# Freebirdgo/MapReduce_Rust

Hardware: AMD Instinct MI355X
Metric: word-count input GB/s (whole node) at 1/2/4/8 MI355X + % of HBM roofline (higher is better)
Workload: dtype u8

## Files before the change

mapreduce_rust_amd/csrc/k_keys.hip:

```cpp
#include <algorithm>
#include <type_traits>

#include "mrg_device.h"
#include "mrg_internal.h"

namespace {

inline dim3 grid_for(uint64_t n, int b = 256) { return dim3((unsigned)((n + b - 1) / b)); }

template <int WG>
__device__ __forceinline__ uint64_t wg_append(unsigned long long *counter, bool pred, uint32_t *s_w,
                                              unsigned long long *s_base) {
    const uint64_t m = __ballot(pred);
    const uint32_t wv = threadIdx.x >> 6, lane = __lane_id();
    if (lane == 0) s_w[wv] = (uint32_t)__popcll(m);
    __syncthreads();
    if (threadIdx.x == 0) {
        uint32_t run = 0;
        for (int w = 0; w < WG / 64; ++w) {
            const uint32_t c = s_w[w];
            s_w[w] = run;
            run += c;
        }
        *s_base = run ? atomicAdd(counter, (unsigned long long)run) : 0ull;
    }
    __syncthreads();
    return *s_base + s_w[wv] + (uint64_t)__popcll(m & mrg_lanemask_lt());
}

constexpr int BA_WG = 1024;
constexpr int BA_NW = BA_WG / 64;
template <bool IDX, bool C32>
constexpr uint32_t ba_cap() { return IDX ? 4096u : (C32 ? 6912u : 6112u); }
constexpr int BA_PROBE = 64;
constexpr int BA_U = 8;
template <bool C32>
constexpr int ba_maxreg() { return C32 ? 512 : 2048; }
constexpr uint32_t BA_QN = 64;
template <bool IDX, bool C32>
constexpr bool ba_queue() { return !IDX && C32; }

#define GASK __attribute__((address_space(1)))
template <class T>
__device__ __forceinline__ GASK T *gk(T *p) {
    return (GASK T *)p;
}
typedef uint64_t u64x2k __attribute__((ext_vector_type(2)));
typedef uint32_t u32x3k __attribute__((ext_vector_type(3), aligned(4)));

__device__ __forceinline__ uint32_t ba_hash(uint64_t a, uint64_t b, uint32_t d, uint32_t hash_bits) {
    uint32_t h = mrg_key_hash32(a, b, d);
    if (hash_bits && hash_bits < 32) h &= (1u << hash_bits) - 1u;
    return h;
}

struct alignas(16) BaKey {
    unsigned long long a, b;
};

template <bool IDX, bool C32>
__device__ __forceinline__ uint32_t ba_slot(uint32_t h) {
    return (((h >> (32 - MRG_NBUCKET_LOG2 - 16)) & 0xFFFFu) * ba_cap<IDX, C32>()) >> 16;
}

template <bool IDX, bool C32, class CT>
__device__ __forceinline__ bool ba_add_from(BaKey *key, CT *cnt, unsigned int *doc, uint64_t a,
                                            uint64_t b, uint32_t d, uint64_t c, uint32_t h, BaKey first) {
    constexpr uint32_t CAP = ba_cap<IDX, C32>();
    uint32_t slot = ba_slot<IDX, C32>(h);
    BaKey kn = first;
    for (int p = 0; p < BA_PROBE; ++p) {
        const BaKey k = kn;
        uint32_t nxt = slot + 1u + (uint32_t)p;
        if (nxt >= CAP) nxt -= CAP;
        kn = key[nxt];
        const bool dk = !IDX || doc[slot] == d;
        if (k.a == a && k.b == b && dk) {
            atomicAdd(&cnt[slot], (CT)c);
            return true;
        }
        if (k.a == MRG_EMPTY_K0 || (k.a == a && (k.b == MRG_EMPTY_K1 || (IDX && k.b == b)))) {
            const unsigned long long x = atomicCAS(&key[slot].a, MRG_EMPTY_K0, (unsigned long long)a);
            if (x == MRG_EMPTY_K0 || x == a) {
                const unsigned long long y = atomicCAS(&key[slot].b, MRG_EMPTY_K1, (unsigned long long)b);
                if (y == MRG_EMPTY_K1 || y == b) {
                    bool ok = true;
                    if (IDX) {
                        const unsigned int z = atomicCAS(&doc[slot], MRG_EMPTY_DOC, d);
                        ok = (z == MRG_EMPTY_DOC || z == d);
                    }
                    if (ok) {
                        atomicAdd(&cnt[slot], (CT)c);
                        return true;
                    }
                }
            }
        }
        slot = nxt;
    }
    return false;
}

template <bool IDX, bool C32, class CT>
__device__ __forceinline__ bool ba_add(BaKey *key, CT *cnt, unsigned int *doc, uint64_t a,
                                       uint64_t b, uint32_t d, uint64_t c, uint32_t h) {
    return ba_add_from<IDX, C32>(key, cnt, doc, a, b, d, c, h, key[ba_slot<IDX, C32>(h)]);
}

#ifndef MRG_AGG_XCD
#define MRG_AGG_XCD 1
#endif
static_assert(MRG_NBUCKET % 8 == 0, "buckets spread over the 8 XCDs");
template <bool IDX, bool C32>
__global__ __launch_bounds__(BA_WG, 1) void k_bucket_agg(BucketArgs A) {
    constexpr uint32_t BA_CAP = ba_cap<IDX, C32>();
    using CT = typename std::conditional<C32, unsigned int, unsigned long long>::type;
    __shared__ BaKey s_key[BA_CAP];
    __shared__ CT s_cnt[BA_CAP];
    __shared__ unsigned int s_doc[IDX ? BA_CAP : 1];
    __shared__ uint32_t s_rn[ba_maxreg<C32>()];
    __shared__ uint32_t s_cs[ba_maxreg<C32>() + 1];
    __shared__ BaKey s_mq[ba_queue<IDX, C32>() ? BA_NW : 1][ba_queue<IDX, C32>() ? BA_QN : 1];
    const int tid = threadIdx.x, lane = tid & 63;
    const int wv = __builtin_amdgcn_readfirstlane(tid >> 6);
    for (int i = tid; i < (int)BA_CAP; i += BA_WG) {
        s_key[i] = BaKey{MRG_EMPTY_K0, MRG_EMPTY_K1};
        s_cnt[i] = 0;
        if (IDX) s_doc[i] = MRG_EMPTY_DOC;
    }
    const uint32_t nsub = A.nsub;
#if MRG_AGG_XCD
    const uint32_t g = blockIdx.x, slot = g / 8u;
    const uint32_t b = nsub > 1u ? (slot / nsub) * 8u + g % 8u : g % MRG_NBUCKET;
    const uint32_t jsub = nsub > 1u ? slot % nsub : g / MRG_NBUCKET;
#else
    const uint32_t b = blockIdx.x % MRG_NBUCKET, jsub = blockIdx.x / MRG_NBUCKET;
#endif
    auto mine = [&](uint32_t h) { return nsub <= 1u || (((h & 0xFFu) * nsub) >> 8) == jsub; };
    constexpr uint32_t RW = IDX ? 3u : 2u;
    const uint32_t cap = gk(A.bcap)[b];
    const uint32_t nreg = A.nreg;
    for (uint32_t r = tid; r < nreg; r += BA_WG) s_rn[r] = min(gk(A.bcount)[(uint64_t)r * MRG_NBUCKET + b], cap);
    __syncthreads();
    constexpr uint32_t CH = 64u * BA_U;
    if (wv == 0) {
        uint32_t run = 0;
        for (uint32_t r0 = 0; r0 < nreg; r0 += 64) {
            const uint32_t r = r0 + (uint32_t)lane;
            const uint32_t c = r < nreg ? (s_rn[r] + CH - 1u) / CH : 0u;
            uint32_t incl = c;
            for (int o = 1; o < 64; o <<= 1) {
                const uint32_t v = __shfl_up(incl, o);
                if (lane >= o) incl += v;
            }
            if (r < nreg) s_cs[r] = run + incl - c;
            run += (uint32_t)__builtin_amdgcn_readlane((int)incl, 63);
        }
        if (lane == 0) s_cs[nreg] = run;
    }
    __syncthreads();
    const uint32_t NC = s_cs[nreg];

    auto overflow = [&](bool ovf, uint64_t a, uint64_t c, uint32_t d, uint64_t n2) {
        const uint64_t j = mrg_wave_append(&A.counters[CNT_OVF2], ovf);
        if (ovf && j < A.ocap) {
            gk(A.ok0)[j] = a; gk(A.ok1)[j] = c; gk(A.ocnt)[j] = (uint32_t)n2;
            if (IDX) gk(A.odoc)[j] = d;
        }
    };

    const GASK uint8_t *pool = reinterpret_cast<const GASK uint8_t *>(gk(A.pool)) + A.rbase[b] * MRG_TAIL_BYTES(IDX);
    struct Chunk {
        u64x2k k[BA_U];
        uint32_t d[IDX ? BA_U : 1];
    };
    auto chunk_pos = [&](uint32_t k, uint32_t &r) -> uint32_t {
        while (s_cs[r + 1] <= k) ++r;
        return (k - s_cs[r]) * CH;
    };
    auto load_chunk = [&](uint32_t r, uint32_t off, Chunk &X) {
        const uint32_t n = s_rn[r];
        const GASK uint8_t *src = pool + (uint64_t)r * cap * MRG_TAIL_BYTES(IDX);
#pragma unroll
        for (int k = 0; k < BA_U; ++k) {
            const uint32_t i = min(off + 64u * k + (uint32_t)lane, n - 1u);
            if (IDX) {
                const GASK uint64_t *rec = reinterpret_cast<const GASK uint64_t *>(src) + (uint64_t)i * 3;
                X.k[k] = u64x2k{rec[0], rec[1]};
                X.d[k] = (uint32_t)rec[2];
            } else {
                const u32x3k v = __builtin_nontemporal_load(reinterpret_cast<const GASK u32x3k *>(src + (uint64_t)i * 12u));
                X.k[k] = u64x2k{(uint64_t)v.x | ((uint64_t)v.y << 32), (uint64_t)v.z << 32};
            }
        }
    };
    auto settle = [](Chunk &X) {
#pragma unroll
        for (int k = 0; k < BA_U; ++k) asm volatile("" : "+v"(X.k[k]));
        if (IDX)
            for (int k = 0; k < BA_U; ++k) asm volatile("" : "+v"(X.d[k]));
    };
    uint64_t abl_acc = 0;
    uint32_t qn = 0;
    auto drain = [&]() {
        if (!ba_queue<IDX, C32>() || qn == 0) return;
        const bool act = (uint32_t)lane < qn;
        const BaKey r = s_mq[ba_queue<IDX, C32>() ? wv : 0][act ? lane : 0];
        bool ovf = false;
        if (act) {
            const uint32_t h = ba_hash(r.a, r.b, MRG_EMPTY_DOC, A.hash_bits);
            ovf = !ba_add<IDX, C32>(s_key, s_cnt, s_doc, r.a, r.b, MRG_EMPTY_DOC, 1ull, h);
        }
        if (__any(ovf)) overflow(ovf, r.a, r.b, MRG_EMPTY_DOC, 1);
        qn = 0;
    };
    auto sum_chunk = [&](uint32_t r, uint32_t off, const Chunk &X) {
        const uint32_t n = s_rn[r];
        if (A.ablate) {
#pragma unroll
            for (int k = 0; k < BA_U; ++k) {
                const bool ok = off + 64u * k + (uint32_t)lane < n;
                const uint64_t a = X.k[k].x, c = X.k[k].y;
                const uint32_t d = IDX ? X.d[k] : MRG_EMPTY_DOC;
                abl_acc += ok ? ((A.ablate & 2u) ? (a ^ c) : (uint64_t)ba_hash(a, c, d, A.hash_bits)) : 0u;
            }
            return;
        }
        uint32_t hk[BA_U];
#pragma unroll
        for (int k = 0; k < BA_U; ++k) hk[k] = ba_hash(X.k[k].x, X.k[k].y, IDX ? X.d[k] : MRG_EMPTY_DOC, A.hash_bits);
        BaKey pre = s_key[ba_slot<IDX, C32>(hk[0])];
        if constexpr (ba_queue<IDX, C32>()) {
#pragma unroll
            for (int k = 0; k < BA_U; ++k) {
                const bool ok = off + 64u * k + (uint32_t)lane < n;
                const uint64_t a = X.k[k].x, c = X.k[k].y;
                const BaKey first = pre;
                if (k + 1 < BA_U) pre = s_key[ba_slot<IDX, C32>(hk[k + 1 < BA_U ? k + 1 : k])];
                const uint32_t h = hk[k];
                const bool me = ok && mine(h);
                const bool hit = me && first.a == a && first.b == c;
                if (hit) atomicAdd(&s_cnt[ba_slot<IDX, C32>(h)], (CT)1);
                const bool miss = me && !hit;
                const uint64_t mm = __ballot(miss);
                if (mm) {
                    const uint32_t m = (uint32_t)__builtin_popcountll(mm);
                    if (qn + m > BA_QN) drain();
                    if (miss) s_mq[wv][qn + (uint32_t)__builtin_popcountll(mm & mrg_lanemask_lt())] = BaKey{a, c};
                    qn += m;
                }
            }
            return;
        }
#pragma unroll
        for (int k = 0; k < BA_U; ++k) {
            const bool ok = off + 64u * k + (uint32_t)lane < n;
            const uint64_t a = X.k[k].x, c = X.k[k].y;
            const uint32_t d = IDX ? X.d[k] : MRG_EMPTY_DOC;
            const BaKey first = pre;
            if (k + 1 < BA_U) pre = s_key[ba_slot<IDX, C32>(hk[k + 1 < BA_U ? k + 1 : k])];
            bool ovf = false;
            const uint32_t h = hk[k];
            if (ok && mine(h)) ovf = !ba_add_from<IDX, C32>(s_key, s_cnt, s_doc, a, c, d, 1ull, h, first);
            if (__any(ovf)) overflow(ovf, a, c, d, 1);
        }
    };
    if (!(A.ablate & 4u)) {
        Chunk XA, XB;
        uint32_t kA = (uint32_t)wv, rA = 0, oA = 0;
        if (kA < NC) {
            oA = chunk_pos(kA, rA);
            load_chunk(rA, oA, XA);
        }
        while (kA < NC) {
            const uint32_t kB = kA + BA_NW;
            uint32_t rB = rA, oB = oA;
            if (kB < NC) oB = chunk_pos(kB, rB);
            settle(XA);
            load_chunk(rB, oB, XB);
            sum_chunk(rA, oA, XA);
            if (kB >= NC) break;
            kA = kB + BA_NW;
            rA = rB;
            if (kA < NC) oA = chunk_pos(kA, rA);
            else oA = oB;
            settle(XB);
            load_chunk(rA, oA, XA);
            sum_chunk(rB, oB, XB);
        }
    }
    drain();

    if (A.ablate && abl_acc == 0x9E3779B97F4A7C15ull) atomicAdd(&A.counters[CNT_OVF2], 1ull);
    {
        const uint32_t nrw = nreg > (uint32_t)wv ? (nreg - (uint32_t)wv + BA_NW - 1) / BA_NW : 0u;
        for (uint32_t l0 = 0; l0 < nrw; l0 += 64) {
            const uint32_t l = l0 + (uint32_t)lane;
            uint32_t lo = 0, cnt = 0;
            if (l < nrw) {
                const GASK uint32_t *fo = gk(A.foff) + (uint64_t)(wv + BA_NW * l) * (MRG_NBUCKET + 1);
                lo = fo[b];
                cnt = fo[b + 1] - lo;
            }
            uint32_t incl = cnt;
            for (int o = 1; o < 64; o <<= 1) {
                const uint32_t v = __shfl_up(incl, o);
                if (lane >= o) incl += v;
            }
            const uint32_t excl = incl - cnt;
            const uint32_t total = (uint32_t)__builtin_amdgcn_readlane((int)incl, 63);
            for (uint32_t e0 = 0; e0 < total; e0 += 256) {
                uint64_t a[4], c[4];
                uint32_t n2[4], d[4];
                bool ok[4];
#pragma unroll
                for (int u = 0; u < 4; ++u) {
                    const uint32_t e = e0 + 64u * u + (uint32_t)lane;
                    ok[u] = e < total;
                    uint32_t k = 0;
#pragma unroll
                    for (int st = 32; st > 0; st >>= 1)
                        if (__shfl(excl, (int)(k + st)) <= e) k += st;
                    const uint32_t rl = l0 + k;
                    const uint64_t at = (uint64_t)(wv + BA_NW * rl) * A.regcap + __shfl(lo, (int)k) + (e - __shfl(excl, (int)k));
                    a[u] = 0; c[u] = 0; n2[u] = 0; d[u] = MRG_EMPTY_DOC;
                    if (ok[u]) {
                        a[u] = gk(A.fk0)[at];
                        c[u] = gk(A.fk1)[at];
                        n2[u] = gk(A.fcnt)[at];
                        if (IDX) d[u] = gk(A.fdoc)[at];
                    }
                }
#pragma unroll
                for (int u = 0; u < 4; ++u) {
                    bool ovf = false;
                    if (ok[u]) {
                        const uint32_t h = ba_hash(a[u], c[u], d[u], A.hash_bits);
                        if (mine(h)) ovf = !ba_add<IDX, C32>(s_key, s_cnt, s_doc, a[u], c[u], d[u], n2[u], h);
                    }
                    if (__any(ovf)) overflow(ovf, a[u], c[u], d[u], n2[u]);
                }
            }
        }
    }
    if (!IDX) {
        const uint32_t cap16 = gk(A.bcap16)[b];
        const GASK uint64_t *p16 = gk(A.pool16) + 2ull * A.rbase16[b];
        for (uint32_t r = (uint32_t)wv; r < nreg; r += BA_NW) {
            const uint32_t n = min(gk(A.bcount16)[(uint64_t)r * MRG_NBUCKET + b], cap16);
            const GASK uint64_t *src = p16 + 2ull * r * cap16;
            for (uint32_t base = 0; base < n; base += 64) {
                const uint32_t i = base + (uint32_t)lane;
                bool ovf = false;
                uint64_t a = 0, c = 0;
                if (i < n) {
                    const u64x2k v = *reinterpret_cast<const GASK u64x2k *>(src + 2ull * i);
                    a = v.x;
                    c = v.y;
                    const uint32_t h = ba_hash(a, c, MRG_EMPTY_DOC, A.hash_bits);
                    if (mine(h)) ovf = !ba_add<IDX, C32>(s_key, s_cnt, s_doc, a, c, MRG_EMPTY_DOC, 1ull, h);
                }
                if (__any(ovf)) overflow(ovf, a, c, MRG_EMPTY_DOC, 1);
            }
        }
    }
    {
        const uint32_t n = min(gk(A.monext)[b], A.mocap);
        const GASK uint64_t *src = gk(A.movf) + (uint64_t)b * A.mocap * RW;
        for (uint32_t base = wv * 64u; base < n; base += BA_WG) {
            const uint32_t i = base + lane;
            bool ovf = false;
            uint64_t a = 0, c = 0;
            uint32_t d = MRG_EMPTY_DOC;
            if (i < n) {
                a = src[(uint64_t)i * RW];
                c = src[(uint64_t)i * RW + 1];
                if (IDX) d = (uint32_t)src[(uint64_t)i * RW + 2];
                const uint32_t h = ba_hash(a, c, d, A.hash_bits);
                if (mine(h)) ovf = !ba_add<IDX, C32>(s_key, s_cnt, s_doc, a, c, d, 1ull, h);
            }
            if (__any(ovf)) overflow(ovf, a, c, d, 1);
        }
    }
    __syncthreads();
    constexpr int NP = (int)((BA_CAP + BA_WG - 1) / BA_WG);
    constexpr int NPW = NP * BA_NW;
    static_assert(NPW <= 128, "one wave scans two entries per lane");
    __shared__ uint32_t s_po[NPW];
    __shared__ unsigned long long s_base;
#pragma unroll
    for (int pp = 0; pp < NP; ++pp) {
        const int i = pp * BA_WG + tid;
        const uint64_t m = __ballot(i < (int)BA_CAP && s_key[min(i, (int)BA_CAP - 1)].a != MRG_EMPTY_K0);
        if (lane == 0) s_po[pp * BA_NW + wv] = (uint32_t)__popcll(m);
    }
    __syncthreads();
    if (wv == 0) {
        const int e0 = 2 * lane, e1 = e0 + 1;
        const uint32_t c0 = e0 < NPW ? s_po[e0] : 0u, c1 = e1 < NPW ? s_po[e1] : 0u;
        uint32_t incl = c0 + c1;
        for (int o = 1; o < 64; o <<= 1) {
            const uint32_t v = __shfl_up(incl, o);
            if (lane >= o) incl += v;
        }
        const uint32_t ex = incl - c0 - c1;
        if (e0 < NPW) s_po[e0] = ex;
        if (e1 < NPW) s_po[e1] = ex + c0;
        const uint32_t tot = (uint32_t)__shfl((int)incl, 63);
        if (lane == 0) s_base = tot ? atomicAdd(&A.counters[CNT_KEYS], (unsigned long long)tot) : 0ull;
    }
    __syncthreads();
    const uint64_t kbase = s_base;
    for (int pp = 0; pp < NP; ++pp) {
        const int i = min(pp * BA_WG + tid, (int)BA_CAP - 1);
        const BaKey k = s_key[i];
        const bool full = pp * BA_WG + tid < (int)BA_CAP && k.a != MRG_EMPTY_K0;
        const uint64_t m = __ballot(full);
        const uint64_t j = kbase + s_po[pp * BA_NW + wv] + (uint64_t)__popcll(m & mrg_lanemask_lt());
        if (full && j < A.kcap) {
            gk(A.out.k0)[j] = k.a;
            gk(A.out.k1)[j] = k.b;
            gk(A.out.cnt)[j] = s_cnt[i];
            gk(A.out.doc)[j] = IDX ? s_doc[i] : MRG_EMPTY_DOC;
            const uint32_t L = mrg_short_len(k.a, k.b);
            gk(A.out.len)[j] = L;
            gk(A.out.hoff)[j] = MRG_NO_HEAP;
            if (A.n_reduce) gk(A.out.part)[j] = (uint32_t)(mrg_siphash_short(k.a, k.b, L) % (uint64_t)A.n_reduce);
        }
    }
}

__global__ __launch_bounds__(1024) void k_stage_scatter(const uint8_t *stage, uint32_t table_off, uint32_t nops) {
    const StageOp *ops = reinterpret_cast<const StageOp *>(stage + table_off);
    for (uint32_t k = 0; k < nops; ++k) {
        const StageOp op = ops[k];
        uint8_t *dst = reinterpret_cast<uint8_t *>(op.dst);
        const bool fill = op.src == 0xFFFFFFFFu;
        if (((op.dst | op.n) & 3u) == 0u) {
            const uint32_t f4 = op.fill * 0x01010101u;
            const uint32_t *src = reinterpret_cast<const uint32_t *>(stage + (fill ? 0u : op.src));
            for (uint32_t i = threadIdx.x; i < op.n / 4u; i += blockDim.x)
                reinterpret_cast<uint32_t *>(dst)[i] = fill ? f4 : src[i];
        } else {
            for (uint32_t i = threadIdx.x; i < op.n; i += blockDim.x) dst[i] = fill ? (uint8_t)op.fill : stage[op.src + i];
        }
        __syncthreads();
    }
}

__global__ void k_table_clear(TableArgs T, bool idx) {
    const uint64_t i = (uint64_t)blockIdx.x * blockDim.x + threadIdx.x;
    if (i >= T.cap) return;
    T.tk0[i] = MRG_EMPTY_K0;
    T.tk1[i] = MRG_EMPTY_K1;
    T.tcnt[i] = 0;
    if (idx) T.tdoc[i] = MRG_EMPTY_DOC;
}

__device__ __forceinline__ void table_add(const TableArgs &T, uint64_t a, uint64_t b, uint32_t d, uint64_t c,
                                          bool idx) {
    uint64_t h = mrg_key_mix(a, b, d);
    if (T.hash_bits) h &= (1ull << T.hash_bits) - 1u;
    uint64_t slot = (h ^ (h >> 31)) & (T.cap - 1);
    for (uint64_t probe = 0; probe < T.cap; ++probe) {
        const unsigned long long x =
            atomicCAS((unsigned long long *)&T.tk0[slot], MRG_EMPTY_K0, (unsigned long long)a);
        if (x == MRG_EMPTY_K0 || x == a) {
            const unsigned long long y =
                atomicCAS((unsigned long long *)&T.tk1[slot], MRG_EMPTY_K1, (unsigned long long)b);
            if (y == MRG_EMPTY_K1 || y == b) {
                bool ok = true;
                if (idx) {
                    const unsigned int z = atomicCAS(&T.tdoc[slot], MRG_EMPTY_DOC, d);
                    ok = (z == MRG_EMPTY_DOC || z == d);
                }
                if (ok) {
                    atomicAdd((unsigned long long *)&T.tcnt[slot], (unsigned long long)c);
                    return;
                }
            }
        }
        slot = (slot + probe + 1u) & (T.cap - 1);
    }
}

__global__ void k_table_insert(TableArgs T, const uint64_t *k0, const uint64_t *k1, const uint32_t *cnt,
                               const uint32_t *doc, uint64_t n, bool idx) {
    const uint64_t i = (uint64_t)blockIdx.x * blockDim.x + threadIdx.x;
    if (i >= n) return;
    table_add(T, k0[i], k1[i], idx ? doc[i] : MRG_EMPTY_DOC, cnt[i], idx);
}

__global__ void k_table_insert_x(TableArgs T, const XRec *x, uint64_t n, bool idx) {
    const uint64_t i = (uint64_t)blockIdx.x * blockDim.x + threadIdx.x;
    if (i >= n) return;
    const XRec r = x[i];
    if (r.len > 16u) return;
    table_add(T, r.a, r.b, idx ? r.v : MRG_EMPTY_DOC, idx ? 1ull : (uint64_t)r.v, idx);
}

__global__ void k_table_insert_l(TableArgs T, const LRec *x, uint64_t n, bool idx) {
    const uint64_t i = (uint64_t)blockIdx.x * blockDim.x + threadIdx.x;
    if (i >= n) return;
    const LRec r = x[i];
    if (r.len > 16u) return;
    table_add(T, r.k0, r.k1, idx ? r.doc : MRG_EMPTY_DOC, r.cnt, idx);
}

constexpr int TC_WG = 1024;
__global__ __launch_bounds__(TC_WG) void k_table_compact(TableArgs T, bool idx, KeySet out, unsigned long long *counter) {
    __shared__ uint32_t s_w[TC_WG / 64];
    __shared__ unsigned long long s_base;
    const uint64_t i = (uint64_t)blockIdx.x * blockDim.x + threadIdx.x;
    const bool full = i < T.cap && T.tk0[i] != MRG_EMPTY_K0;
    const uint64_t j = wg_append<TC_WG>(counter, full, s_w, &s_base);
    if (!full) return;
    const uint64_t a = T.tk0[i], b = T.tk1[i];
    out.k0[j] = a;
    out.k1[j] = b;
    out.cnt[j] = T.tcnt[i];
    out.doc[j] = idx ? T.tdoc[i] : MRG_EMPTY_DOC;
    out.len[j] = mrg_short_len(a, b);
    out.hoff[j] = MRG_NO_HEAP;
}

__global__ void k_partition(KeySet ks, const uint8_t *heap, uint64_t n, uint32_t n_reduce) {
    const uint64_t i = (uint64_t)blockIdx.x * blockDim.x + threadIdx.x;
    if (i >= n) return;
    const uint32_t L = ks.len[i];
    const uint64_t h = L <= 16u ? mrg_siphash_short(ks.k0[i], ks.k1[i], L) : mrg_siphash_bytes(heap + ks.hoff[i], L);
    ks.part[i] = (uint32_t)(h % (uint64_t)n_reduce);
}

__global__ void k_wide_counts(BucketArgs A, uint64_t *cnt) {
    const uint64_t s = (uint64_t)blockIdx.x * blockDim.x + threadIdx.x;
    const uint64_t nt = (uint64_t)A.nreg * MRG_NBUCKET;
    if (s < nt) {
        const uint32_t b = (uint32_t)(s / A.nreg), w = (uint32_t)(s % A.nreg);
        cnt[s] = min(A.bcount[(uint64_t)w * MRG_NBUCKET + b], A.bcap[b]);
    } else if (s < nt + A.nreg) {
        const uint64_t w = s - nt;
        cnt[s] = A.foff[w * (MRG_NBUCKET + 1) + MRG_NBUCKET];
    } else if (s < nt + A.nreg + MRG_NBUCKET) {
        const uint32_t b = (uint32_t)(s - nt - A.nreg);
        cnt[s] = min(A.monext[b], A.mocap);
    } else if (s < 2 * nt + A.nreg + MRG_NBUCKET) {
        const uint64_t s2 = s - nt - A.nreg - MRG_NBUCKET;
        const uint32_t b = (uint32_t)(s2 / A.nreg), w = (uint32_t)(s2 % A.nreg);
        cnt[s] = min(A.bcount16[(uint64_t)w * MRG_NBUCKET + b], A.bcap16[b]);
    }
}

__global__ void k_wide_gather(BucketArgs A, const uint64_t *off, uint32_t n_reduce, SortRec *out) {
    const uint64_t s = blockIdx.x;
    const uint64_t nt = (uint64_t)A.nreg * MRG_NBUCKET;
    const uint64_t o = off[s], n = off[s + 1] - o;
    for (uint64_t i = threadIdx.x; i < n; i += blockDim.x) {
        uint64_t k0, k1;
        uint32_t c = 1;
        if (s < nt) {
            const uint32_t b = (uint32_t)(s / A.nreg), w = (uint32_t)(s % A.nreg);
            const uint64_t j = A.rbase[b] + (uint64_t)w * A.bcap[b] + i;
            const uint32_t *rec = reinterpret_cast<const uint32_t *>(reinterpret_cast<const uint8_t *>(A.pool) + 12u * j);
            k0 = (uint64_t)rec[0] | ((uint64_t)rec[1] << 32);
            k1 = (uint64_t)rec[2] << 32;
        } else if (s >= nt + A.nreg + MRG_NBUCKET) {
            const uint64_t s2 = s - nt - A.nreg - MRG_NBUCKET;
            const uint32_t b = (uint32_t)(s2 / A.nreg), w = (uint32_t)(s2 % A.nreg);
            const uint64_t j = A.rbase16[b] + (uint64_t)w * A.bcap16[b] + i;
            k0 = A.pool16[2 * j];
            k1 = A.pool16[2 * j + 1];
        } else if (s < nt + A.nreg) {
            const uint64_t j = (s - nt) * A.regcap + i;
            k0 = A.fk0[j];
            k1 = A.fk1[j];
            c = A.fcnt[j];
        } else {
            const uint64_t b = s - nt - A.nreg;
            const uint64_t j = b * A.mocap + i;
            k0 = A.movf[2 * j];
            k1 = A.movf[2 * j + 1];
        }
        SortRec r;
        r.k0 = k0;
        r.k1 = k1;
        r.part = (uint32_t)(mrg_siphash_short(k0, k1, mrg_short_len(k0, k1)) % (uint64_t)n_reduce);
        r.doc = 0;
        r.idx = c;
        r.pad = 0;
        out[o + i] = r;
    }
}

__global__ void k_wide_heads(const SortRec *r, uint64_t n, uint64_t *head, uint64_t *cv) {
    const uint64_t i = (uint64_t)blockIdx.x * blockDim.x + threadIdx.x;
    if (i >= n) return;
    head[i] = (i == 0 || r[i].k0 != r[i - 1].k0 || r[i].k1 != r[i - 1].k1) ? 1u : 0u;
    cv[i] = r[i].idx;
}

__global__ void k_wide_keys(const SortRec *r, uint64_t n, const uint64_t *head, const uint64_t *E, KeySet ks,
                            uint64_t *F) {
    const uint64_t i = (uint64_t)blockIdx.x * blockDim.x + threadIdx.x;
    if (i >= n || !head[i]) return;
    const uint64_t k = E[i];
    ks.k0[k] = r[i].k0;
    ks.k1[k] = r[i].k1;
    ks.doc[k] = MRG_EMPTY_DOC;
    ks.len[k] = mrg_short_len(r[i].k0, r[i].k1);
    ks.part[k] = r[i].part;
    ks.hoff[k] = MRG_NO_HEAP;
    F[k] = i;
}

__global__ void k_wide_cnt(const uint64_t *F, uint64_t runs, uint64_t n, const uint64_t *C, uint64_t ctot, KeySet ks) {
    const uint64_t k = (uint64_t)blockIdx.x * blockDim.x + threadIdx.x;
    if (k >= runs) return;
    const uint64_t e = k + 1 < runs ? C[F[k + 1]] : ctot;
    ks.cnt[k] = e - C[F[k]];
}

__global__ void k_long_group(const uint64_t *fp, const uint32_t *idx, const uint32_t *doc, const uint8_t *heap,
                             const uint64_t *hoff, const uint32_t *flen, uint64_t n, uint32_t *rep) {
    const uint64_t i = (uint64_t)blockIdx.x * blockDim.x + threadIdx.x;
    if (i >= n) return;
    const uint32_t me = idx[i];
    const uint64_t f = fp[i];
    uint64_t g = 0, hi = i;
    while (g < hi) {
        const uint64_t mid = (g + hi) >> 1;
        if (fp[mid] < f) g = mid + 1; else hi = mid;
    }
    uint32_t r = me;
    const uint8_t *mk = heap + hoff[me];
    const uint32_t ml = flen[me];
    for (uint64_t j = g; j < i; ++j) {
        const uint32_t o = idx[j];
        if (flen[o] != ml || (doc && doc[o] != doc[me])) continue;
        const uint8_t *ok = heap + hoff[o];
        bool eq = true;
        for (uint32_t b = 0; b < ml && eq; ++b) eq = mk[b] == ok[b];
        if (eq) { r = o; break; }
    }
    rep[me] = r;
}

__global__ void k_long_count(const uint32_t *rep, const uint64_t *cnt_in, uint64_t n, unsigned long long *acc) {
    const uint64_t i = (uint64_t)blockIdx.x * blockDim.x + threadIdx.x;
    if (i >= n) return;
    atomicAdd(&acc[rep[i]], (unsigned long long)(cnt_in ? cnt_in[i] : 1u));
}

__global__ void k_long_emit(const uint32_t *rep, const uint64_t *k0, const uint64_t *k1, const uint32_t *flen,
                            const uint64_t *hoff, const uint32_t *doc, uint64_t n, const unsigned long long *acc,
                            KeySet out, unsigned long long *counter, bool idx) {
    const uint64_t i = (uint64_t)blockIdx.x * blockDim.x + threadIdx.x;
    const bool mine = i < n && rep[i] == (uint32_t)i;
    const uint64_t j = mrg_wave_append(counter, mine);
    if (!mine) return;
    out.k0[j] = k0[i];
    out.k1[j] = k1[i];
    out.cnt[j] = acc[i];
    out.doc[j] = idx ? doc[i] : MRG_EMPTY_DOC;
    out.len[j] = flen[i];
    out.hoff[j] = hoff[i];
}

__device__ __forceinline__ uint32_t seg_of(const uint64_t *seg_rec_end, uint32_t n_segs, uint64_t i) {
    uint32_t lo = 0, hi = n_segs - 1u;
    while (lo < hi) {
        const uint32_t mid = (lo + hi) >> 1;
        if (i < seg_rec_end[mid]) hi = mid;
        else lo = mid + 1u;
    }
    return lo;
}

__global__ void k_x_split_long(const XRec *x, uint64_t n, const uint64_t *seg_rec_end, const uint64_t *seg_heap_base,
                               uint32_t n_segs, LongItems li, unsigned long long *counter, bool idx) {
    const uint64_t i = (uint64_t)blockIdx.x * blockDim.x + threadIdx.x;
    const bool lng = i < n && x[i].len > 16u;
    const uint64_t j = mrg_wave_append(counter, lng);
    if (!lng) return;
    const XRec r = x[i];
    li.start[j] = seg_heap_base[seg_of(seg_rec_end, n_segs, i)] + r.a;
    li.rawlen[j] = r.len;
    li.doc[j] = idx ? r.v : MRG_EMPTY_DOC;
    li.cnt[j] = idx ? 1ull : r.b;
}

__global__ void k_l_split_long(const LRec *x, uint64_t n, const uint64_t *seg_rec_end, const uint64_t *seg_heap_base,
                               uint32_t n_segs, LongItems li, unsigned long long *counter) {
    const uint64_t i = (uint64_t)blockIdx.x * blockDim.x + threadIdx.x;
    const bool lng = i < n && x[i].len > 16u;
    const uint64_t j = mrg_wave_append(counter, lng);
    if (!lng) return;
    const LRec r = x[i];
    li.start[j] = seg_heap_base[seg_of(seg_rec_end, n_segs, i)] + r.heap;
    li.rawlen[j] = r.len;
    li.doc[j] = r.doc;
    li.cnt[j] = r.cnt;
}

constexpr int EXP_WG = 1024;
constexpr uint32_t EXP_MAXO = 256;

__global__ __launch_bounds__(EXP_WG) void k_export_count(KeySet ks, uint64_t n, uint32_t n_owners,
                                                         unsigned long long *rec_cnt, unsigned long long *heap_cnt,
                                                         bool idx, uint64_t vmax) {
    __shared__ unsigned long long s_rc[EXP_MAXO];
    __shared__ unsigned long long s_hc[EXP_MAXO];
    const bool lds = n_owners <= EXP_MAXO;
    if (lds)
        for (uint32_t o = threadIdx.x; o < n_owners; o += EXP_WG) {
            s_rc[o] = 0;
            s_hc[o] = 0;
        }
    __syncthreads();
    const uint64_t i = (uint64_t)blockIdx.x * blockDim.x + threadIdx.x;
    if (i < n) {
        const uint32_t o = ks.part[i] % n_owners;
        const uint32_t len = ks.len[i];
        const unsigned long long nr = mrg_xrec_per_key(ks.cnt[i], len, idx, vmax);
        if (lds) {
            atomicAdd(&s_rc[o], nr);
            if (len > 16u) atomicAdd(&s_hc[o], (unsigned long long)len);
        } else {
            atomicAdd(&rec_cnt[o], nr);
            if (len > 16u) atomicAdd(&heap_cnt[o], (unsigned long long)len);
        }
    }
    if (!lds) return;
    __syncthreads();
    for (uint32_t o = threadIdx.x; o < n_owners; o += EXP_WG) {
        if (s_rc[o]) atomicAdd(&rec_cnt[o], (unsigned long long)s_rc[o]);
        if (s_hc[o]) atomicAdd(&heap_cnt[o], s_hc[o]);
    }
}

__global__ __launch_bounds__(EXP_WG) void k_export_pack(KeySet ks, const uint8_t *heap, uint64_t n, uint32_t n_owners,
                                                        const uint64_t *rec_base, const uint64_t *heap_base,
                                                        unsigned long long *rec_cur, unsigned long long *heap_cur,
                                                        XRec *out, uint8_t *out_heap, bool idx, uint64_t vmax) {
    __shared__ unsigned long long s_rc[EXP_MAXO];
    __shared__ unsigned long long s_hc[EXP_MAXO], s_rb[EXP_MAXO], s_hb[EXP_MAXO];
    const bool lds = n_owners <= EXP_MAXO;
    if (lds)
        for (uint32_t o = threadIdx.x; o < n_owners; o += EXP_WG) {
            s_rc[o] = 0;
            s_hc[o] = 0;
        }
    __syncthreads();
    const uint64_t i = (uint64_t)blockIdx.x * blockDim.x + threadIdx.x;
    const bool act = i < n;
    uint32_t o = 0, len = 0;
    uint64_t cnt = 0, nr = 0;
    unsigned long long lr = 0, lh = 0;
    if (act) {
        o = ks.part[i] % n_owners;
        len = ks.len[i];
        cnt = ks.cnt[i];
        nr = mrg_xrec_per_key(cnt, len, idx, vmax);
        if (lds) {
            lr = atomicAdd(&s_rc[o], (unsigned long long)nr);
            if (len > 16u) lh = atomicAdd(&s_hc[o], (unsigned long long)len);
        } else {
            lr = atomicAdd(&rec_cur[o], (unsigned long long)nr);
            if (len > 16u) lh = atomicAdd(&heap_cur[o], (unsigned long long)len);
        }
    }
    if (lds) {
        __syncthreads();
        for (uint32_t q = threadIdx.x; q < n_owners; q += EXP_WG) {
            s_rb[q] = s_rc[q] ? atomicAdd(&rec_cur[q], (unsigned long long)s_rc[q]) : 0ull;
            s_hb[q] = s_hc[q] ? atomicAdd(&heap_cur[q], s_hc[q]) : 0ull;
        }
        __syncthreads();
        if (act) {
            lr += s_rb[o];
            lh += s_hb[o];
        }
    }
    if (!act) return;
    const uint64_t slot = rec_base[o] + lr;
    XRec r;
    r.len = len;
    if (len > 16u) {
        const uint8_t *src = heap + ks.hoff[i];
        uint8_t *dst = out_heap + heap_base[o] + lh;
        for (uint32_t b = 0; b < len; ++b) dst[b] = src[b];
        r.a = lh;
        r.b = idx ? 1ull : cnt;
        r.v = idx ? ks.doc[i] : MRG_EMPTY_DOC;
        out[slot] = r;
        return;
    }
    r.a = ks.k0[i];
    r.b = ks.k1[i];
    if (idx) {
        r.v = ks.doc[i];
        out[slot] = r;
        return;
    }
    for (uint64_t k = 0; k < nr; ++k) {
        const uint64_t c = cnt > vmax ? vmax : cnt;
        cnt -= c;
        r.v = (uint32_t)c;
        out[slot + k] = r;
    }
}

__global__ void k_make_sortrec(KeySet ks, uint64_t n, const uint32_t *doc_rank, SortRec *out, int carry) {
    const uint64_t i = (uint64_t)blockIdx.x * blockDim.x + threadIdx.x;
    if (i >= n) return;
    SortRec r;
    r.k0 = ks.k0[i];
    r.k1 = ks.k1[i];
    r.part = ks.part[i];
    r.doc = doc_rank ? doc_rank[ks.doc[i]] : 0u;
    r.idx = (uint32_t)i;
    r.pad = 0;
    if (carry) {
        const uint64_t c = ks.cnt[i];
        const uint32_t len = ks.len[i];
        r.doc = (uint32_t)c;
        r.pad = (len <= 16u ? len : 0xFFu) | ((uint32_t)(c >> 32) << 8);
    }
    out[i] = r;
}

template <class T>
__global__ void k_fill(T *p, T v, uint64_t n) {
    const uint64_t i = (uint64_t)blockIdx.x * blockDim.x + threadIdx.x;
    if (i < n) p[i] = v;
}
__global__ void k_iota(uint32_t *p, uint64_t n) {
    const uint64_t i = (uint64_t)blockIdx.x * blockDim.x + threadIdx.x;
    if (i < n) p[i] = (uint32_t)i;
}

}

void mrg_launch_stage_scatter(const uint8_t *d_stage, uint32_t table_off, uint32_t nops, hipStream_t s) {
    if (nops) hipLaunchKernelGGL(k_stage_scatter, dim3(1), dim3(1024), 0, s, d_stage, table_off, nops);
}

void mrg_launch_bucket_agg(const BucketArgs &a, bool indexer, bool count32, hipStream_t s) {
    const dim3 g(MRG_NBUCKET * std::max<uint32_t>(a.nsub, 1u));
    if (indexer) hipLaunchKernelGGL((k_bucket_agg<true, false>), g, dim3(BA_WG), 0, s, a);
    else if (count32) hipLaunchKernelGGL((k_bucket_agg<false, true>), g, dim3(BA_WG), 0, s, a);
    else hipLaunchKernelGGL((k_bucket_agg<false, false>), g, dim3(BA_WG), 0, s, a);
}

void mrg_launch_table_clear(const TableArgs &t, bool indexer, hipStream_t s) {
    hipLaunchKernelGGL(k_table_clear, grid_for(t.cap), dim3(256), 0, s, t, indexer);
}
void mrg_launch_table_insert(const TableArgs &t, const uint64_t *k0, const uint64_t *k1, const uint32_t *cnt32,
                             const uint32_t *doc, uint64_t n, bool indexer, hipStream_t s) {
    if (!n) return;
    hipLaunchKernelGGL(k_table_insert, grid_for(n), dim3(256), 0, s, t, k0, k1, cnt32, doc, n, indexer);
}
void mrg_launch_table_insert_x(const TableArgs &t, const XRec *x, uint64_t n, bool indexer, hipStream_t s) {
    if (!n) return;
    hipLaunchKernelGGL(k_table_insert_x, grid_for(n), dim3(256), 0, s, t, x, n, indexer);
}
void mrg_launch_table_insert_l(const TableArgs &t, const LRec *x, uint64_t n, bool indexer, hipStream_t s) {
    if (!n) return;
    hipLaunchKernelGGL(k_table_insert_l, grid_for(n), dim3(256), 0, s, t, x, n, indexer);
}
void mrg_launch_table_compact(const TableArgs &t, bool indexer, KeySet out, unsigned long long *counter,
                              hipStream_t s) {
    hipLaunchKernelGGL(k_table_compact, grid_for(t.cap, TC_WG), dim3(TC_WG), 0, s, t, indexer, out, counter);
}
void mrg_launch_partition(KeySet ks, const uint8_t *heap, uint64_t n, uint32_t n_reduce, hipStream_t s) {
    if (!n) return;
    hipLaunchKernelGGL(k_partition, grid_for(n), dim3(256), 0, s, ks, heap, n, n_reduce);
}
void mrg_launch_long_group(const uint64_t *fp_sorted, const uint32_t *idx_sorted, const uint32_t *doc,
                           const uint8_t *heap, const uint64_t *hoff, const uint32_t *flen, uint64_t n,
                           uint32_t *rep, hipStream_t s) {
    if (!n) return;
    hipLaunchKernelGGL(k_long_group, grid_for(n), dim3(256), 0, s, fp_sorted, idx_sorted, doc, heap, hoff, flen, n,
                       rep);
}
void mrg_launch_long_emit(const uint32_t *rep, const uint64_t *cnt_in, const uint64_t *k0, const uint64_t *k1,
                          const uint32_t *flen, const uint64_t *hoff, const uint32_t *doc, uint64_t n,
                          unsigned long long *acc, KeySet out, unsigned long long *counter, bool indexer,
                          hipStream_t s) {
    if (!n) return;
    hipLaunchKernelGGL(k_long_count, grid_for(n), dim3(256), 0, s, rep, cnt_in, n, acc);
    hipLaunchKernelGGL(k_long_emit, grid_for(n), dim3(256), 0, s, rep, k0, k1, flen, hoff, doc, n,
                       (const unsigned long long *)acc, out, counter, indexer);
}
void mrg_launch_x_split_long(const XRec *x, uint64_t n, const uint64_t *seg_rec_end, const uint64_t *seg_heap_base,
                             uint32_t n_segs, LongItems li, unsigned long long *counter, bool indexer, hipStream_t s) {
    if (!n) return;
    hipLaunchKernelGGL(k_x_split_long, grid_for(n), dim3(256), 0, s, x, n, seg_rec_end, seg_heap_base, n_segs, li,
                       counter, indexer);
}
void mrg_launch_l_split_long(const LRec *x, uint64_t n, const uint64_t *seg_rec_end, const uint64_t *seg_heap_base,
                             uint32_t n_segs, LongItems li, unsigned long long *counter, hipStream_t s) {
    if (!n) return;
    hipLaunchKernelGGL(k_l_split_long, grid_for(n), dim3(256), 0, s, x, n, seg_rec_end, seg_heap_base, n_segs, li,
                       counter);
}
void mrg_launch_export_count(KeySet ks, uint64_t n, uint32_t n_owners, unsigned long long *rec_cnt,
                             unsigned long long *heap_cnt, bool indexer, uint64_t vmax, hipStream_t s) {
    if (!n) return;
    hipLaunchKernelGGL(k_export_count, grid_for(n, EXP_WG), dim3(EXP_WG), 0, s, ks, n, n_owners, rec_cnt, heap_cnt,
                       indexer, vmax);
}
void mrg_launch_export_pack(KeySet ks, const uint8_t *heap, uint64_t n, uint32_t n_owners,
                            const uint64_t *rec_base, const uint64_t *heap_base, unsigned long long *rec_cur,
                            unsigned long long *heap_cur, XRec *out, uint8_t *out_heap, bool indexer, uint64_t vmax,
                            hipStream_t s) {
    if (!n) return;
    hipLaunchKernelGGL(k_export_pack, grid_for(n, EXP_WG), dim3(EXP_WG), 0, s, ks, heap, n, n_owners, rec_base,
                       heap_base, rec_cur, heap_cur, out, out_heap, indexer, vmax);
}
void mrg_launch_make_sortrec(KeySet ks, uint64_t n, const uint32_t *doc_rank, void *recs, hipStream_t s, bool carry) {
    if (!n) return;
    hipLaunchKernelGGL(k_make_sortrec, grid_for(n), dim3(256), 0, s, ks, n, doc_rank, (SortRec *)recs, carry ? 1 : 0);
}
void mrg_launch_wide_counts(const BucketArgs &a, uint64_t *cnt, uint64_t nseg, hipStream_t s) {
    hipLaunchKernelGGL(k_wide_counts, grid_for(nseg), dim3(256), 0, s, a, cnt);
}
void mrg_launch_wide_gather(const BucketArgs &a, const uint64_t *off, uint64_t nseg, uint32_t n_reduce, SortRec *out,
                            hipStream_t s) {
    hipLaunchKernelGGL(k_wide_gather, dim3((unsigned)nseg), dim3(256), 0, s, a, off, n_reduce, out);
}
void mrg_launch_wide_heads(const SortRec *r, uint64_t n, uint64_t *head, uint64_t *cv, hipStream_t s) {
    if (n) hipLaunchKernelGGL(k_wide_heads, grid_for(n), dim3(256), 0, s, r, n, head, cv);
}
void mrg_launch_wide_keys(const SortRec *r, uint64_t n, const uint64_t *head, const uint64_t *E, KeySet ks,
                          uint64_t *F, hipStream_t s) {
    if (n) hipLaunchKernelGGL(k_wide_keys, grid_for(n), dim3(256), 0, s, r, n, head, E, ks, F);
}
void mrg_launch_wide_cnt(const uint64_t *F, uint64_t runs, uint64_t n, const uint64_t *C, uint64_t ctot, KeySet ks,
                         hipStream_t s) {
    if (runs) hipLaunchKernelGGL(k_wide_cnt, grid_for(runs), dim3(256), 0, s, F, runs, n, C, ctot, ks);
}
void mrg_launch_fill_u32(uint32_t *p, uint32_t v, uint64_t n, hipStream_t s) {
    if (!n) return;
    hipLaunchKernelGGL(k_fill<uint32_t>, grid_for(n), dim3(256), 0, s, p, v, n);
}
void mrg_launch_fill_u64(uint64_t *p, uint64_t v, uint64_t n, hipStream_t s) {
    if (!n) return;
    hipLaunchKernelGGL(k_fill<uint64_t>, grid_for(n), dim3(256), 0, s, p, v, n);
}
void mrg_launch_iota_u32(uint32_t *p, uint64_t n, hipStream_t s) {
    if (!n) return;
    hipLaunchKernelGGL(k_iota, grid_for(n), dim3(256), 0, s, p, n);
}
```

Before: 1521.

## Deepen bucket-agg load pipeline and batch miss-queue probing in word-count aggregation

For the non-index path, the bucket aggregation kernel now keeps three chunk loads in flight instead of two, with five records per lane per chunk instead of eight. Queued misses are drained through a new wave-batched probe that issues four shared-memory slot loads per round trip before comparing. Per-bucket metadata (bcount, foff, bcount16, monext) is fetched before the shared-table initialisation so its latency overlaps the clears. The bcount16 pass now skips empty regions using a ballot over counts. The aim is to hide global-memory and LDS latency, at the cost of more registers and extra wasted probe loads.

```diff
diff --git a/mapreduce_rust_amd/csrc/k_keys.hip b/mapreduce_rust_amd/csrc/k_keys.hip
--- a/mapreduce_rust_amd/csrc/k_keys.hip
+++ b/mapreduce_rust_amd/csrc/k_keys.hip
@@ -33,7 +33,16 @@
 template <bool IDX, bool C32>
 constexpr uint32_t ba_cap() { return IDX ? 4096u : (C32 ? 6912u : 6112u); }
 constexpr int BA_PROBE = 64;
-constexpr int BA_U = 8;
+#ifndef MRG_AGG_U
+#define MRG_AGG_U 5
+#endif
+#ifndef MRG_AGG_DEPTH
+#define MRG_AGG_DEPTH 3
+#endif
+template <bool IDX>
+constexpr int ba_u() { return IDX ? 8 : MRG_AGG_U; }
+template <bool IDX>
+constexpr int ba_depth() { return IDX ? 2 : MRG_AGG_DEPTH; }
 template <bool C32>
 constexpr int ba_maxreg() { return C32 ? 512 : 2048; }
 constexpr uint32_t BA_QN = 64;
@@ -52,6 +61,10 @@
     uint32_t h = mrg_key_hash32(a, b, d);
     if (hash_bits && hash_bits < 32) h &= (1u << hash_bits) - 1u;
     return h;
+}
+
+__device__ __forceinline__ uint32_t ba_rank(uint64_t m) {
+    return __builtin_amdgcn_mbcnt_hi((uint32_t)(m >> 32), __builtin_amdgcn_mbcnt_lo((uint32_t)m, 0u));
 }
 
 struct alignas(16) BaKey {
@@ -107,6 +120,46 @@
     return ba_add_from<IDX, C32>(key, cnt, doc, a, b, d, c, h, key[ba_slot<IDX, C32>(h)]);
 }
 
+template <bool C32, class CT>
+__device__ __forceinline__ bool ba_add_wave(BaKey *key, CT *cnt, uint64_t a, uint64_t b, uint32_t h, bool act) {
+    constexpr uint32_t CAP = ba_cap<false, C32>();
+    constexpr int W = 4;
+    static_assert(BA_PROBE % W == 0, "whole round trips");
+    uint32_t slot = ba_slot<false, C32>(h);
+    bool todo = act;
+    for (int p0 = 0; p0 < BA_PROBE && __any(todo); p0 += W) {
+        if (todo) {
+            uint32_t s[W];
+            BaKey k[W];
+#pragma unroll
+            for (int j = 0; j < W; ++j) {
+                s[j] = slot;
+                k[j] = key[slot];
+                slot += 1u + (uint32_t)(p0 + j);
+                if (slot >= CAP) slot -= CAP;
+            }
+#pragma unroll
+            for (int j = 0; j < W; ++j) {
+                if (!todo) continue;
+                if (k[j].a == a && k[j].b == b) {
+                    atomicAdd(&cnt[s[j]], (CT)1);
+                    todo = false;
+                } else if (k[j].a == MRG_EMPTY_K0 || (k[j].a == a && k[j].b == MRG_EMPTY_K1)) {
+                    const unsigned long long x = atomicCAS(&key[s[j]].a, MRG_EMPTY_K0, (unsigned long long)a);
+                    if (x == MRG_EMPTY_K0 || x == a) {
+                        const unsigned long long y = atomicCAS(&key[s[j]].b, MRG_EMPTY_K1, (unsigned long long)b);
+                        if (y == MRG_EMPTY_K1 || y == b) {
+                            atomicAdd(&cnt[s[j]], (CT)1);
+                            todo = false;
+                        }
+                    }
+                }
+            }
+        }
+    }
+    return !todo;
+}
+
 #ifndef MRG_AGG_XCD
 #define MRG_AGG_XCD 1
 #endif
@@ -114,6 +167,7 @@
 template <bool IDX, bool C32>
 __global__ __launch_bounds__(BA_WG, 1) void k_bucket_agg(BucketArgs A) {
     constexpr uint32_t BA_CAP = ba_cap<IDX, C32>();
+    constexpr int BA_U = ba_u<IDX>(), BA_D = ba_depth<IDX>();
     using CT = typename std::conditional<C32, unsigned int, unsigned long long>::type;
     __shared__ BaKey s_key[BA_CAP];
     __shared__ CT s_cnt[BA_CAP];
@@ -123,11 +177,6 @@
     __shared__ BaKey s_mq[ba_queue<IDX, C32>() ? BA_NW : 1][ba_queue<IDX, C32>() ? BA_QN : 1];
     const int tid = threadIdx.x, lane = tid & 63;
     const int wv = __builtin_amdgcn_readfirstlane(tid >> 6);
-    for (int i = tid; i < (int)BA_CAP; i += BA_WG) {
-        s_key[i] = BaKey{MRG_EMPTY_K0, MRG_EMPTY_K1};
-        s_cnt[i] = 0;
-        if (IDX) s_doc[i] = MRG_EMPTY_DOC;
-    }
     const uint32_t nsub = A.nsub;
 #if MRG_AGG_XCD
     const uint32_t g = blockIdx.x, slot = g / 8u;
@@ -140,7 +189,27 @@
     constexpr uint32_t RW = IDX ? 3u : 2u;
     const uint32_t cap = gk(A.bcap)[b];
     const uint32_t nreg = A.nreg;
-    for (uint32_t r = tid; r < nreg; r += BA_WG) s_rn[r] = min(gk(A.bcount)[(uint64_t)r * MRG_NBUCKET + b], cap);
+    const uint32_t nrw = nreg > (uint32_t)wv ? (nreg - (uint32_t)wv + BA_NW - 1) / BA_NW : 0u;
+    const uint32_t rn0 = (uint32_t)tid < nreg ? gk(A.bcount)[(uint64_t)tid * MRG_NBUCKET + b] : 0u;
+    uint32_t fo_lo0 = 0, fo_hi0 = 0, n16_0 = 0, movf_n = 0;
+    auto fetch_ends = [&]() {
+        if ((uint32_t)lane < nrw) {
+            const uint64_t r = (uint64_t)(wv + BA_NW * lane);
+            const GASK uint32_t *fo = gk(A.foff) + r * (MRG_NBUCKET + 1);
+            fo_lo0 = fo[b];
+            fo_hi0 = fo[b + 1];
+            if (!IDX) n16_0 = gk(A.bcount16)[r * MRG_NBUCKET + b];
+        }
+        movf_n = min(gk(A.monext)[b], A.mocap);
+    };
+    if (!IDX) fetch_ends();
+    for (int i = tid; i < (int)BA_CAP; i += BA_WG) {
+        s_key[i] = BaKey{MRG_EMPTY_K0, MRG_EMPTY_K1};
+        s_cnt[i] = 0;
+        if (IDX) s_doc[i] = MRG_EMPTY_DOC;
+    }
+    if ((uint32_t)tid < nreg) s_rn[tid] = min(rn0, cap);
+    for (uint32_t r = tid + BA_WG; r < nreg; r += BA_WG) s_rn[r] = min(gk(A.bcount)[(uint64_t)r * MRG_NBUCKET + b], cap);
     __syncthreads();
     constexpr uint32_t CH = 64u * BA_U;
     if (wv == 0) {
@@ -161,7 +230,7 @@
     __syncthreads();
     const uint32_t NC = s_cs[nreg];
 
-    auto overflow = [&](bool ovf, uint64_t a, uint64_t c, uint32_t d, uint64_t n2) {
+    auto overflow = [&](bool ovf, uint64_t a, uint64_t c, uint32_t d, uint64_t n2) __attribute__((always_inline)) {
         const uint64_t j = mrg_wave_append(&A.counters[CNT_OVF2], ovf);
         if (ovf && j < A.ocap) {
             gk(A.ok0)[j] = a; gk(A.ok1)[j] = c; gk(A.ocnt)[j] = (uint32_t)n2;
@@ -202,19 +271,18 @@
     };
     uint64_t abl_acc = 0;
     uint32_t qn = 0;
-    auto drain = [&]() {
-        if (!ba_queue<IDX, C32>() || qn == 0) return;
-        const bool act = (uint32_t)lane < qn;
-        const BaKey r = s_mq[ba_queue<IDX, C32>() ? wv : 0][act ? lane : 0];
-        bool ovf = false;
-        if (act) {
+    auto drain = [&]() __attribute__((always_inline)) {
+        if constexpr (ba_queue<IDX, C32>()) {
+            if (qn == 0) return;
+            const bool act = (uint32_t)lane < qn;
+            const BaKey r = s_mq[wv][act ? lane : 0];
             const uint32_t h = ba_hash(r.a, r.b, MRG_EMPTY_DOC, A.hash_bits);
-            ovf = !ba_add<IDX, C32>(s_key, s_cnt, s_doc, r.a, r.b, MRG_EMPTY_DOC, 1ull, h);
-        }
-        if (__any(ovf)) overflow(ovf, r.a, r.b, MRG_EMPTY_DOC, 1);
-        qn = 0;
+            const bool ovf = act && !ba_add_wave<C32>(s_key, s_cnt, r.a, r.b, h, act);
+            if (__any(ovf)) overflow(ovf, r.a, r.b, MRG_EMPTY_DOC, 1);
+            qn = 0;
+        }
     };
-    auto sum_chunk = [&](uint32_t r, uint32_t off, const Chunk &X) {
+    auto sum_chunk = [&](uint32_t r, uint32_t off, const Chunk &X) __attribute__((always_inline)) {
         const uint32_t n = s_rn[r];
         if (A.ablate) {
 #pragma unroll
@@ -231,24 +299,36 @@
         for (int k = 0; k < BA_U; ++k) hk[k] = ba_hash(X.k[k].x, X.k[k].y, IDX ? X.d[k] : MRG_EMPTY_DOC, A.hash_bits);
         BaKey pre = s_key[ba_slot<IDX, C32>(hk[0])];
         if constexpr (ba_queue<IDX, C32>()) {
+            const uint32_t left = n - min(n, off + (uint32_t)lane);
+            uint32_t pend = 0;
 #pragma unroll
             for (int k = 0; k < BA_U; ++k) {
-                const bool ok = off + 64u * k + (uint32_t)lane < n;
                 const uint64_t a = X.k[k].x, c = X.k[k].y;
                 const BaKey first = pre;
                 if (k + 1 < BA_U) pre = s_key[ba_slot<IDX, C32>(hk[k + 1 < BA_U ? k + 1 : k])];
                 const uint32_t h = hk[k];
-                const bool me = ok && mine(h);
+                bool me = 64u * k < left;
+                if (nsub > 1u) {
+                    asm volatile("");
+                    me = me && mine(h);
+                }
                 const bool hit = me && first.a == a && first.b == c;
                 if (hit) atomicAdd(&s_cnt[ba_slot<IDX, C32>(h)], (CT)1);
-                const bool miss = me && !hit;
-                const uint64_t mm = __ballot(miss);
-                if (mm) {
+                if (me && !hit) pend |= 1u << k;
+            }
+            while (__any(pend != 0u)) {
+#pragma unroll
+                for (int k = 0; k < BA_U; ++k) {
+                    const bool miss = (pend >> k) & 1u;
+                    const uint64_t mm = __ballot(miss);
                     const uint32_t m = (uint32_t)__builtin_popcountll(mm);
-                    if (qn + m > BA_QN) drain();
-                    if (miss) s_mq[wv][qn + (uint32_t)__builtin_popcountll(mm & mrg_lanemask_lt())] = BaKey{a, c};
-                    qn += m;
+                    if (mm && qn + m <= BA_QN) {
+                        if (miss) s_mq[wv][qn + ba_rank(mm)] = BaKey{X.k[k].x, X.k[k].y};
+                        qn += m;
+                        pend &= ~(1u << k);
+                    }
                 }
+                if (__any(pend != 0u)) drain();
             }
             return;
         }
@@ -265,39 +345,69 @@
             if (__any(ovf)) overflow(ovf, a, c, d, 1);
         }
     };
-    if (!(A.ablate & 4u)) {
-        Chunk XA, XB;
-        uint32_t kA = (uint32_t)wv, rA = 0, oA = 0;
-        if (kA < NC) {
-            oA = chunk_pos(kA, rA);
-            load_chunk(rA, oA, XA);
-        }
-        while (kA < NC) {
-            const uint32_t kB = kA + BA_NW;
-            uint32_t rB = rA, oB = oA;
-            if (kB < NC) oB = chunk_pos(kB, rB);
-            settle(XA);
-            load_chunk(rB, oB, XB);
-            sum_chunk(rA, oA, XA);
-            if (kB >= NC) break;
-            kA = kB + BA_NW;
-            rA = rB;
-            if (kA < NC) oA = chunk_pos(kA, rA);
-            else oA = oB;
-            settle(XB);
-            load_chunk(rA, oA, XA);
-            sum_chunk(rB, oB, XB);
+    if constexpr (BA_D == 2) {
+        if (!(A.ablate & 4u)) {
+            Chunk XA, XB;
+            uint32_t kA = (uint32_t)wv, rA = 0, oA = 0;
+            if (kA < NC) {
+                oA = chunk_pos(kA, rA);
+                load_chunk(rA, oA, XA);
+            }
+            while (kA < NC) {
+                const uint32_t kB = kA + BA_NW;
+                uint32_t rB = rA, oB = oA;
+                if (kB < NC) oB = chunk_pos(kB, rB);
+                settle(XA);
+                load_chunk(rB, oB, XB);
+                sum_chunk(rA, oA, XA);
+                if (kB >= NC) break;
+                kA = kB + BA_NW;
+                rA = rB;
+                if (kA < NC) oA = chunk_pos(kA, rA);
+                else oA = oB;
+                settle(XB);
+                load_chunk(rA, oA, XA);
+                sum_chunk(rB, oB, XB);
+            }
+        }
+    } else if (!(A.ablate & 4u) && (uint32_t)wv < NC) {
+        Chunk X[BA_D];
+        uint32_t rr[BA_D], oo[BA_D];
+        uint32_t k = (uint32_t)wv;
+        rr[0] = 0;
+        oo[0] = chunk_pos(k, rr[0]);
+        load_chunk(rr[0], oo[0], X[0]);
+        auto next = [&](uint32_t kk, int from, int to) {
+            rr[to] = rr[from];
+            oo[to] = kk < NC ? chunk_pos(kk, rr[to]) : oo[from];
+        };
+#pragma unroll
+        for (int j = 1; j < BA_D - 1; ++j) {
+            next(k + (uint32_t)j * BA_NW, j - 1, j);
+            load_chunk(rr[j], oo[j], X[j]);
+        }
+        while (k < NC) {
+#pragma unroll
+            for (int j = 0; j < BA_D; ++j) {
+                constexpr int D1 = BA_D - 1;
+                next(k + (uint32_t)D1 * BA_NW, (j + BA_D - 2) % BA_D, (j + D1) % BA_D);
+                settle(X[j]);
+                load_chunk(rr[(j + D1) % BA_D], oo[(j + D1) % BA_D], X[(j + D1) % BA_D]);
+                sum_chunk(rr[j], oo[j], X[j]);
+                k += BA_NW;
+                if (k >= NC) break;
+            }
         }
     }
     drain();
 
     if (A.ablate && abl_acc == 0x9E3779B97F4A7C15ull) atomicAdd(&A.counters[CNT_OVF2], 1ull);
     {
-        const uint32_t nrw = nreg > (uint32_t)wv ? (nreg - (uint32_t)wv + BA_NW - 1) / BA_NW : 0u;
+        if (IDX) fetch_ends();
         for (uint32_t l0 = 0; l0 < nrw; l0 += 64) {
             const uint32_t l = l0 + (uint32_t)lane;
-            uint32_t lo = 0, cnt = 0;
-            if (l < nrw) {
+            uint32_t lo = l0 ? 0u : fo_lo0, cnt = l0 ? 0u : fo_hi0 - fo_lo0;
+            if (l0 && l < nrw) {
                 const GASK uint32_t *fo = gk(A.foff) + (uint64_t)(wv + BA_NW * l) * (MRG_NBUCKET + 1);
                 lo = fo[b];
                 cnt = fo[b + 1] - lo;
@@ -346,26 +456,34 @@
     if (!IDX) {
         const uint32_t cap16 = gk(A.bcap16)[b];
         const GASK uint64_t *p16 = gk(A.pool16) + 2ull * A.rbase16[b];
-        for (uint32_t r = (uint32_t)wv; r < nreg; r += BA_NW) {
-            const uint32_t n = min(gk(A.bcount16)[(uint64_t)r * MRG_NBUCKET + b], cap16);
-            const GASK uint64_t *src = p16 + 2ull * r * cap16;
-            for (uint32_t base = 0; base < n; base += 64) {
-                const uint32_t i = base + (uint32_t)lane;
-                bool ovf = false;
-                uint64_t a = 0, c = 0;
-                if (i < n) {
-                    const u64x2k v = *reinterpret_cast<const GASK u64x2k *>(src + 2ull * i);
-                    a = v.x;
-                    c = v.y;
-                    const uint32_t h = ba_hash(a, c, MRG_EMPTY_DOC, A.hash_bits);
-                    if (mine(h)) ovf = !ba_add<IDX, C32>(s_key, s_cnt, s_doc, a, c, MRG_EMPTY_DOC, 1ull, h);
+        for (uint32_t l0 = 0; l0 < nrw; l0 += 64) {
+            const uint32_t l = l0 + (uint32_t)lane;
+            uint32_t n16 = n16_0;
+            if (l0) n16 = l < nrw ? gk(A.bcount16)[(uint64_t)(wv + BA_NW * l) * MRG_NBUCKET + b] : 0u;
+            n16 = min(n16, cap16);
+            for (uint64_t live = __ballot(n16 != 0u); live; live &= live - 1) {
+                const int k = __builtin_ctzll(live);
+                const uint32_t n = (uint32_t)__shfl((int)n16, k);
+                const uint32_t r = (uint32_t)wv + BA_NW * (l0 + (uint32_t)k);
+                const GASK uint64_t *src = p16 + 2ull * r * cap16;
+                for (uint32_t base = 0; base < n; base += 64) {
+                    const uint32_t i = base + (uint32_t)lane;
+                    bool ovf = false;
+                    uint64_t a = 0, c = 0;
+                    if (i < n) {
+                        const u64x2k v = *reinterpret_cast<const GASK u64x2k *>(src + 2ull * i);
+                        a = v.x;
+                        c = v.y;
+                        const uint32_t h = ba_hash(a, c, MRG_EMPTY_DOC, A.hash_bits);
+                        if (mine(h)) ovf = !ba_add<IDX, C32>(s_key, s_cnt, s_doc, a, c, MRG_EMPTY_DOC, 1ull, h);
+                    }
+                    if (__any(ovf)) overflow(ovf, a, c, MRG_EMPTY_DOC, 1);
                 }
-                if (__any(ovf)) overflow(ovf, a, c, MRG_EMPTY_DOC, 1);
             }
         }
     }
     {
-        const uint32_t n = min(gk(A.monext)[b], A.mocap);
+        const uint32_t n = movf_n;
         const GASK uint64_t *src = gk(A.movf) + (uint64_t)b * A.mocap * RW;
         for (uint32_t base = wv * 64u; base < n; base += BA_WG) {
             const uint32_t i = base + lane;
```

Result: no change. 1536, median of 6 (+0.9%).
